# nyx-ai/droneRL

Hardware: AMD Instinct MI355X
Metric: env-steps/sec (obs/s) at num_envs=65536, 1/2/4/8 MI355X; %HBM roofline (higher is better)
Workload: dtype u8

## Files before the change

dronerl_amd/csrc/dronerl_internal.h:

```cpp
#pragma once
#include <hip/hip_runtime.h>
#include <stdint.h>

#include "../../include/dronerl.h"

namespace drl {

constexpr int MT_N = 624;
constexpr int MT_M = 397;
constexpr int MT_WORDS = DRL_MT_WORDS;
constexpr int MT_ALT = DRL_MT_BLOCK1;
constexpr int MT_RING = DRL_MT_RING;
constexpr int CAND_Q = DRL_CAND_SLOTS;
constexpr int MT_RING_END = DRL_MT_RING_END;
static_assert((CAND_Q & (CAND_Q - 1)) == 0 && CAND_Q <= 512, "ring size");
static_assert(MT_RING_END < MT_WORDS && MT_RING + CAND_Q <= MT_RING_END && MT_WORDS % 16 == 0, "MT row layout");

__host__ __device__ constexpr int mi_idx(uint32_t w) { return (int)(w & 0x3ffu); }
__host__ __device__ constexpr int mi_par(uint32_t w) { return (int)((w >> 10) & 1u); }
__host__ __device__ constexpr int mi_head(uint32_t w) { return (int)((w >> 11) & (uint32_t)(CAND_Q - 1)); }
__host__ __device__ constexpr int mi_cnt(uint32_t w) {
    return (int)((w >> 20) & 0x3ffu) < CAND_Q ? (int)((w >> 20) & 0x3ffu) : CAND_Q;
}
__host__ __device__ constexpr uint32_t mi_pack(int idx, int par, int head, int cnt) {
    return (uint32_t)idx | ((uint32_t)par << 10) | ((uint32_t)head << 11) | ((uint32_t)cnt << 20);
}
__host__ __device__ constexpr int ce_cell(uint32_t e) { return (int)(e & 0x3fffu); }
__host__ __device__ constexpr int ce_idx(uint32_t e) { return (int)((e >> 16) & 0x3ffu); }
__host__ __device__ constexpr int ce_par(uint32_t e) { return (int)((e >> 26) & 1u); }
__host__ __device__ constexpr uint32_t ce_pack(int cell, int idx, int par) {
    return (uint32_t)cell | ((uint32_t)idx << 16) | ((uint32_t)par << 26);
}
#ifndef DRL_CQ_NARROW
#define DRL_CQ_NARROW 2
#endif
constexpr int step_cq(int P) { return P <= 16 ? DRL_CQ_NARROW : 1; }
#ifndef DRL_DPP8
#define DRL_DPP8 1
#endif
#ifndef DRL_DRAWS_P8
#define DRL_DRAWS_P8 2
#endif
#ifndef DRL_DRAWS_P16
#define DRL_DRAWS_P16 2
#endif
#ifndef DRL_DRAWS_P32
#define DRL_DRAWS_P32 1
#endif
constexpr int step_draws(int P) {
    return P == 8 ? DRL_DRAWS_P8 : P == 16 ? DRL_DRAWS_P16 : P == 32 ? DRL_DRAWS_P32 : 1;
}
constexpr int kRolloutMinLanes = 16;
constexpr int kRolloutNoObsMinLanes = 8;
#ifndef DRL_ROLL_RING
#define DRL_ROLL_RING 1
#endif
#ifndef DRL_ROLL_RING_MAXP
#define DRL_ROLL_RING_MAXP 16
#endif
constexpr int OBS_U = 1;

namespace lay {
constexpr int r16(int v) { return (v + 15) / 16 * 16; }
constexpr int np(int n_drones) { return (n_drones + 7) / 8 * 8; }
constexpr int pstride(int side) { return r16((side * side + 1) / 2); }
constexpr int gstride(int side) { return 2 * pstride(side); }
#ifndef DRL_GL_NIB_MIN_SIDE
#define DRL_GL_NIB_MIN_SIDE 32
#endif
constexpr bool gl_nib(int side) { return side >= DRL_GL_NIB_MIN_SIDE; }
constexpr int glstride(int side) { return gl_nib(side) ? pstride(side) : gstride(side); }
constexpr int bm_bytes(int cells) { return r16((cells + 31) / 32 * 4); }
constexpr int paint_bytes(int k, int w) { return k > 0 ? r16(k * w * w) : 0; }
constexpr int nchg(int n_drones) { return 6 * n_drones + 2; }
constexpr int chg_bytes(int n_drones) { return r16(2 * nchg(n_drones)); }
constexpr int bit_length(int v) { return v ? 1 + bit_length(v >> 1) : 0; }
#ifndef DRL_QN_RING
#define DRL_QN_RING 2
#endif
#ifndef DRL_QN_WAVES
#define DRL_QN_WAVES 8
#endif
constexpr int code_cpg(int W) { return (W * W + 3) / 4; }
constexpr int code_cpg8(int W) { return (code_cpg(W) + 7) / 8 * 8; }
constexpr int code_bytes(int W) { return 4 * code_cpg8(W) * 2; }
constexpr int code_slot_cell(int cpg, int sl) { return sl < 6 * (cpg & ~1) ? 2 * (sl / 12) + (sl & 1) : cpg - 1; }
constexpr int code_slot_ch(int cpg, int sl) { return sl < 6 * (cpg & ~1) ? (sl % 12) / 2 : sl - 6 * (cpg - 1); }
constexpr int code_kt(int W) { return ((6 * code_cpg(W) + 7) / 8 + DRL_QN_RING - 1) / DRL_QN_RING * DRL_QN_RING; }
constexpr int qn_ring = DRL_QN_RING;
constexpr int qn_waves = DRL_QN_WAVES;
#ifndef DRL_QN_TILES
#define DRL_QN_TILES 2
#endif
constexpr int qn_tiles = DRL_QN_TILES;
constexpr int fy_bitmap_words(int cells) {
    int w = 64;
    while (w * 32 < cells) w *= 2;
    return w;
}
}

enum : int { OBJ_EMPTY = 0, OBJ_SKYSCRAPER = 2, OBJ_STATION = 3, OBJ_DROPZONE = 4, OBJ_PACKET = 5 };

struct FastDiv {
    uint32_t m;
    int one;
};

inline FastDiv make_fastdiv(uint32_t d) {
    FastDiv f;
    f.one = (d == 1);
    f.m = f.one ? 0u : (uint32_t)((((uint64_t)1 << 32) + d - 1) / d);
    return f;
}

struct ObsGeom {
    int side, radius;
    uint32_t W, per, env_floats, gstride;
    FastDiv div_env, div_per, div_6, div_w, div_side;
};

struct StepArgs {
    int side, n_drones, gstride, kbits;
    int pstride, gl_nib;
    int charge, discharge;
    float r_pickup, r_delivery, r_crash, r_charge;
    int64_t E;
    uint8_t* ground;
    uint32_t* drones;
    uint32_t* mt;
    uint32_t* mt_index;
    const int32_t* actions;
    float* rewards;
    uint8_t* dones;
    float* obs;
    int32_t* err;
    int wave_lds;
    int np;
    int lds_bm;
    int lds_paint;
    int lds_chg;
    int nchg;
    int obs_k;
    int obs_wide;
    int obs_nt;
    int specialize;
    int dones_packed;
    uint4* code;
    int code_lds;
    uint4* ring_obs;
    uint4* ring_next;
    int32_t* ring_act;
    float* ring_rew;
    uint8_t* ring_done;
    const uint4* code_prev;
    int64_t ring_first, ring_base, ring_cap;
    int synth;
    int64_t env_offset;
    uint64_t synth_seed, synth_step;
    uint32_t max_rounds;
    FastDiv div_side;
    ObsGeom og;
    int steps;
    int64_t act_tstride, out_tstride, obs_tstride;
};

struct RefillArgs {
    int side, kbits;
    int list;
    int64_t E;
    uint32_t* mt;
    uint32_t* mt_index;
};

struct ResetArgs {
    int side, n_drones, cells, gstride;
    int n_sky, n_pack, n_drop, n_stat;
    int64_t E;
    uint8_t* ground;
    uint32_t* drones;
    uint32_t* mt;
    uint32_t* mt_index;
    int reseed;
    uint64_t seed_base;
    const uint8_t* mask;
    int lanes, lane_lds, list_cap, block_lds, pool_branch;
    int wave_per_env, wave_lds;
    int wpb;
    int fy_batch_min;
    int fy_serial;
    int fy_bwords;
    FastDiv div_side;
};

constexpr int QN_MAX_LAYERS = 4;
struct QnetLayout {
    int n_layers;
    int nt[QN_MAX_LAYERS];
    int kt[QN_MAX_LAYERS];
    int in[QN_MAX_LAYERS], out[QN_MAX_LAYERS];
    int frag_off[QN_MAX_LAYERS];
    int bias_off[QN_MAX_LAYERS];
    int frag_total;
    int n_bias;
    int lds_vec;
    int precision;
    int frag_lo_off[QN_MAX_LAYERS];
    int total_vec;
    int frag_src[QN_MAX_LAYERS];
    int bias_vec;
    int lo0_lds;
    int code_w;
    int status_vec;
};

struct QnetPack {
    int n_layers;
    int frag_off[QN_MAX_LAYERS], kt[QN_MAX_LAYERS], in[QN_MAX_LAYERS], out[QN_MAX_LAYERS];
    int bias_off[QN_MAX_LAYERS];
    const float* w[QN_MAX_LAYERS];
    const float* b[QN_MAX_LAYERS];
    int64_t n_wfrag_elems, n_bias;
    uint16_t* packed_w;
    float* packed_b;
    int precision;
    int frag_lo_off[QN_MAX_LAYERS];
    int frag_src[QN_MAX_LAYERS];
    int code_w;
    int32_t* status;
};

struct QnetArgs {
    int in_features, kt0, n_hidden, n_actions, precision;
    const float* eps_ptr;
    int nt[QN_MAX_LAYERS];
    int frag_off[QN_MAX_LAYERS], bias_off[QN_MAX_LAYERS];
    int frag_total, lds_vec, n_bias;
    int frag_lo_off[QN_MAX_LAYERS];
    int bias_vec, lo0_lds;
    const uint4* packed;
    const float* obs;
    int64_t obs_stride, E;
    float epsilon;
    uint64_t seed, step;
    int64_t env_offset;
    int32_t* actions;
    int64_t action_stride;
    float* q;
    int synth_n;
    uint64_t synth_seed, synth_step;
    int32_t* err;
    int total_bytes;
    int status_vec;
};

struct ReplayArgs {
    int64_t first, n, cursor, capacity;
    int64_t base;
    int obs_floats;
    const float* obs;
    int64_t obs_stride;
    const float* next_obs;
    int64_t next_obs_stride;
    const int32_t* actions;
    int64_t action_stride;
    const float* rewards;
    int64_t reward_stride;
    const uint8_t* dones;
    int64_t done_stride;
    float* buf_obs;
    float* buf_next_obs;
    int32_t* buf_actions;
    float* buf_rewards;
    uint8_t* buf_dones;
};

__host__ __device__ constexpr int qn_frag_k(int g, int j) { return j < 4 ? 4 * g + j : 16 + 4 * g + (j - 4); }

struct PackSlot {
    int row, k;
};
__host__ __device__ inline PackSlot qnet_pack_slot(int l, int64_t e, int kt, int code_w, int in) {
    const int j = (int)(e & 7), lane = (int)((e >> 3) & 63);
    const int64_t frag = e >> 9;
    const int m = (int)(frag / kt), t = (int)(frag % kt);
    const int c = lane & 15, g = lane >> 4;
    PackSlot s{16 * m + c, 32 * t + qn_frag_k(g, j)};
    if (l == 0 && code_w > 0) {
        const int cpg = lay::code_cpg(code_w), cells = code_w * code_w, sl = 8 * t + j;
        const int lc = lay::code_slot_cell(cpg, sl), ch = lay::code_slot_ch(cpg, sl);
        const bool ok = sl < 6 * cpg && lc < cpg && g * cpg + lc < cells;
        s.k = ok ? (g * cpg + lc) * 6 + ch : in;
        if (g == 0 && sl == 6 * cpg) s.k = -1;
    }
    return s;
}

__host__ __device__ inline int64_t qnet_pack_elem(int l, int row, int k, int kt, int code_w) {
    int t, j, g;
    if (l == 0 && code_w > 0) {
        const int cpg = lay::code_cpg(code_w);
        int sl;
        if (k < 0) {
            g = 0;
            sl = 6 * cpg;
        } else {
            const int cell = k / 6, ch = k - 6 * cell;
            g = (cell >= cpg) + (cell >= 2 * cpg) + (cell >= 3 * cpg);
            const int lc = cell - g * cpg;
            sl = lc < (cpg & ~1) ? 12 * (lc / 2) + 2 * ch + (lc & 1) : 6 * (cpg - 1) + ch;
        }
        t = sl / 8;
        j = sl % 8;
    } else {
        t = k / 32;
        const int kk = k % 32;
        g = kk < 16 ? kk / 4 : (kk - 16) / 4;
        j = kk < 16 ? kk % 4 : 4 + (kk - 16) % 4;
    }
    const int m = row / 16, c = row % 16;
    return (((int64_t)m * kt + t) * 64 + (g * 16 + c)) * 8 + j;
}

__device__ __forceinline__ void qnet_pack_store(const QnetPack& p, int l, int64_t e, float w) {
    if (p.precision == DRL_QNET_F32) {
        if (!(__builtin_fabsf(w) < 65504.0f)) atomicOr(p.status, DRL_ERR_QNET_RANGE);
        const _Float16 hi = (_Float16)w;
        reinterpret_cast<_Float16*>(p.packed_w)[(int64_t)p.frag_off[l] * 8 + e] = hi;
        reinterpret_cast<_Float16*>(p.packed_w)[(int64_t)p.frag_lo_off[l] * 8 + e] = (_Float16)((w - (float)hi) * 2048.0f);
    } else {
        reinterpret_cast<__bf16*>(p.packed_w)[(int64_t)p.frag_off[l] * 8 + e] = (__bf16)w;
    }
}
__device__ __forceinline__ void qnet_pack_write(const QnetPack& p, int l, int64_t e, int k, float w) {
    if (l == 0 && p.code_w > 0 && k >= 0 && k < p.in[l] && k % 6 == 4) w /= 100.0f;
    qnet_pack_store(p, l, e, w);
}
__device__ __forceinline__ void qnet_pack_write_idx(const QnetPack& p, int l, uint32_t pe, float w) {
    if (pe >> 31) w /= 100.0f;
// ... 122 lines not shown
```

dronerl_amd/csrc/dronerl_kernels.hip:

```cpp
#include <hip/hip_runtime.h>
#include <stdint.h>

#include "dronerl_internal.h"
#include "dronerl_act_common.h"

namespace drl {

#ifdef DRL_STAMPS
__device__ unsigned long long* g_stamps;
#define DRL_STAMP(i)                                                                     \
    do {                                                                                 \
        __builtin_amdgcn_sched_barrier(0);                                               \
        unsigned long long t_;                                                           \
        asm volatile("s_memtime %0\n\ts_waitcnt lgkmcnt(0)" : "=s"(t_)::"memory");        \
        const int64_t sw_ = (int64_t)blockIdx.x * (blockDim.x >> 6) + (threadIdx.x >> 6); \
        if ((threadIdx.x & 63) == 0 && g_stamps) g_stamps[sw_ * 16 + (i)] = t_;          \
        if ((threadIdx.x & 63) == 0 && g_stamps && ((i) == 0 || (i) == 6))               \
            g_stamps[sw_ * 16 + 8 + (i) / 6] = __builtin_amdgcn_s_memrealtime();         \
        __builtin_amdgcn_sched_barrier(0);                                               \
    } while (0)
#define DRL_SUBT(v)                                                                  \
    do {                                                                             \
        __builtin_amdgcn_sched_barrier(0);                                           \
        asm volatile("s_memtime %0\n\ts_waitcnt lgkmcnt(0)" : "=s"(v)::"memory");   \
// ... 287 lines not shown
__device__ __forceinline__ uint32_t nib_get(const uint8_t* row, int cell) {
    return (row[cell >> 1] >> ((cell & 1) * 4)) & 15u;
}
__device__ __forceinline__ void nib_or(uint8_t* row, int cell, uint32_t code) {
    atomicOr(reinterpret_cast<uint32_t*>(row) + (cell >> 3), code << ((cell & 7) * 4));
}
__device__ __forceinline__ uint32_t nib_get_l2(uint8_t* row, int cell) {
    const uint32_t w = __hip_atomic_load(reinterpret_cast<uint32_t*>(row) + (cell >> 3), __ATOMIC_RELAXED,
                                         __HIP_MEMORY_SCOPE_AGENT);
    return (w >> ((cell & 7) * 4)) & 15u;
}
__device__ __forceinline__ void nib_clear(uint8_t* row, int cell) {
    atomicAnd(reinterpret_cast<uint32_t*>(row) + (cell >> 3), ~(15u << ((cell & 7) * 4)));
}

template <class GEO>
__device__ __forceinline__ int gl_get(const GEO& g, const l_u8* gl, int cell) {
    if (g.nib()) return (gl[cell >> 1] >> ((cell & 1) << 2)) & 15;
    return gl[cell];
}
template <class GEO>
__device__ __forceinline__ void gl_clear(const GEO& g, l_u8* gl, int cell) {
    if (g.nib()) __atomic_fetch_and(reinterpret_cast<l_u32*>(gl) + (cell >> 3), ~(15u << ((cell & 7) << 2)),
                                    __ATOMIC_RELAXED);
    else gl[cell] = OBJ_EMPTY;
}
template <class GEO>
__device__ __forceinline__ void gl_put(const GEO& g, l_u8* gl, int cell, int obj) {
    if (g.nib()) __atomic_fetch_or(reinterpret_cast<l_u32*>(gl) + (cell >> 3), (uint32_t)obj << ((cell & 7) << 2),
                                   __ATOMIC_RELAXED);
    else gl[cell] = (uint8_t)obj;
}

template <bool NT>
__device__ __forceinline__ void store_obs16(uint4* p, u32x4 v) {
    if constexpr (NT) {
        __builtin_nontemporal_store(v, reinterpret_cast<u32x4*>(p));
    } else {
        *reinterpret_cast<u32x4*>(p) = v;
    }
}

template <class T>
__device__ __forceinline__ void lds_zero(T* p, int nbytes, int lane) {
    l_u4* q = reinterpret_cast<l_u4*>(p);
    for (int v = lane; v < nbytes / 16; v += 64) q[v] = (u32x4){0u, 0u, 0u, 0u};
}

template <bool NT = false, bool CODE = false, bool F32 = true, class GEO>
__device__ __forceinline__ void write_obs_wave(float* __restrict__ base, int nenv_w, const GEO& g, const WaveLds& w,
                                               bool obs_wide, int lane, uint16_t* __restrict__ code = nullptr,
                                               l_u16* cst = nullptr) {
    static_assert(CODE || F32, "nothing to write");
    const uint32_t W = g.W();
    const uint32_t win = W * W;
    const uint32_t env_cells = g.env_cells();
    const uint32_t ncell = (uint32_t)nenv_w * env_cells;
    const int G = g.side(), R = g.radius();
    const uint32_t gstride = (uint32_t)g.gstride(), np = (uint32_t)g.np(), lpaint = (uint32_t)g.lds_paint();
    const bool wide = obs_wide && ((uintptr_t)base & 15u) == 0;
    const int cpg = lay::code_cpg((int)W), cpg8 = lay::code_cpg8((int)W);
    if constexpr (CODE) {
        lds_zero(cst, nenv_w * 8 * cpg8, lane);
        wave_sync();
    }
    for (uint32_t q0 = 0; q0 < ncell; q0 += 64 * OBS_U) {
        uint32_t e[OBS_U], rem[OBS_U], wy[OBS_U], wx[OBS_U], pos[OBS_U];
#pragma unroll
        for (int u = 0; u < OBS_U; ++u) {
            const uint32_t q = min(q0 + (uint32_t)(lane + 64 * u), ncell - 1u);
            e[u] = g.div_env(q);
            rem[u] = q - e[u] * env_cells;
            const uint32_t k = g.div_win(rem[u]);
            const uint32_t c = rem[u] - k * win;
            wy[u] = g.div_w(c);
            wx[u] = c - wy[u] * W;
            pos[u] = w.posidx[e[u] * np + k];
        }
        float2 v[OBS_U][3];
#pragma unroll
        for (int u = 0; u < OBS_U; ++u) {
            const uint32_t py = g.div_side(pos[u]);
            const uint32_t px = pos[u] - py * (uint32_t)G;
            const int y = (int)(py + wy[u]) - R;
            const int x = (int)(px + wx[u]) - R;
            const bool in = (unsigned)y < (unsigned)G && (unsigned)x < (unsigned)G;
            const uint32_t o = (uint32_t)gl_get(g, w.gl + e[u] * gstride, in ? y * G + x : 0);
            const uint32_t obj = in ? o : (uint32_t)OBJ_SKYSCRAPER;
            const uint32_t air = w.paint[e[u] * lpaint + rem[u]];
            if constexpr (CODE) {
                if (rem[u] < win) {
                    const uint32_t cl = rem[u], grpc = cl / (uint32_t)cpg;
                    cst[e[u] * (uint32_t)(4 * cpg8) + grpc * (uint32_t)(cpg8 - cpg) + cl] = (uint16_t)(obj | (air << 3));
                }
            }
            if constexpr (!F32) continue;
            v[u][0].x = air ? 1.0f : 0.0f;
            v[u][0].y = (obj == OBJ_PACKET || (air & 0x80u)) ? 1.0f : 0.0f;
            v[u][1].x = obj == OBJ_DROPZONE ? 1.0f : 0.0f;
            v[u][1].y = obj == OBJ_STATION ? 1.0f : 0.0f;
            v[u][2].x = air ? div100((int)(air & 0x7fu) - 1) : 0.0f;
            v[u][2].y = obj == OBJ_SKYSCRAPER ? 1.0f : 0.0f;
        }
        if constexpr (!F32) continue;
        if (wide) {
            l_f2* st = reinterpret_cast<l_f2*>(w.stage);
#pragma unroll
            for (int u = 0; u < OBS_U; ++u) {
                const int slot = (u * 64 + lane) * 3;
                st[slot] = (f32x2){v[u][0].x, v[u][0].y};
                st[slot + 1] = (f32x2){v[u][1].x, v[u][1].y};
                st[slot + 2] = (f32x2){v[u][2].x, v[u][2].y};
            }
            wave_sync();
            const l_u4* sv = reinterpret_cast<const l_u4*>(w.stage);
            uint4* dst = reinterpret_cast<uint4*>(base + 6u * q0);
            if (q0 + 64u * OBS_U <= ncell) {
#pragma unroll
                for (int t = 0; t < 96 * OBS_U; t += 64)
                    if (96 * OBS_U - t >= 64 || lane < 96 * OBS_U - t) store_obs16<NT>(&dst[t + lane], sv[t + lane]);
            } else {
                const uint32_t nbytes = (ncell - q0) * 24u;
                for (uint32_t t = lane; t * 16u < nbytes; t += 64) {
                    if (t * 16u + 16u <= nbytes) {
                        store_obs16<NT>(&dst[t], sv[t]);
                    } else {
                        reinterpret_cast<u32x2*>(dst + t)[0] = reinterpret_cast<const l_u2*>(sv + t)[0];
                    }
                }
            }
            wave_sync();
        } else {
#pragma unroll
            for (int u = 0; u < OBS_U; ++u) {
                const uint32_t q = q0 + (uint32_t)(lane + 64 * u);
                if (q < ncell) {
                    float2* o = reinterpret_cast<float2*>(base + 6u * q);
                    o[0] = v[u][0];
                    o[1] = v[u][1];
                    o[2] = v[u][2];
                }
            }
        }
    }
    if constexpr (CODE) {
        wave_sync();
        const l_u4* cv = reinterpret_cast<const l_u4*>(cst);
        uint4* dst = reinterpret_cast<uint4*>(code);
        for (int v = lane; v < nenv_w * cpg8 / 2; v += 64) {
            const u32x4 x = cv[v];
            dst[v] = make_uint4(x[0], x[1], x[2], x[3]);
        }
    }
}

template <class GEO>
__device__ __forceinline__ uint16_t* code_row(const StepArgs& a, int64_t wenv0, const GEO& g) {
    return reinterpret_cast<uint16_t*>(a.code) + wenv0 * (int64_t)(4 * lay::code_cpg8((int)g.W()));
}

template <class A>
__device__ __forceinline__ int64_t step_ring_slot(const A& a, int64_t e) {
    const int64_t s = a.ring_base + (e - a.ring_first);
    return s >= a.ring_cap ? s - a.ring_cap : s;
}

template <class A>
__device__ __forceinline__ bool ring_vec(const A& a, int64_t wenv0, uint32_t v, uint32_t VR, int64_t* e,
                                         uint32_t* col) {
    const uint32_t el = v / VR;
    *col = v - el * VR;
    *e = wenv0 + el;
    return *e >= a.ring_first;
}

template <int RQ, class A>
__device__ __forceinline__ void step_ring_prefetch(const A& a, int64_t wenv0, int nenv_w, int lane, uint32_t VR,
                                                   u32x4 (&pre)[RQ]) {
    const uint32_t nv = (uint32_t)nenv_w * VR;
#pragma unroll
    for (int q = 0; q < RQ; ++q) {
        const uint32_t v = (uint32_t)(lane + 64 * q);
        int64_t e;
        uint32_t col;
        if (v < nv && ring_vec(a, wenv0, v, VR, &e, &col))
            pre[q] = reinterpret_cast<const u32x4*>(a.code_prev)[e * VR + col];
    }
}

template <int RQ, class A>
__device__ __forceinline__ void step_ring_sink(const A& a, int64_t wenv0, int nenv_w, const l_u16* cst,
                                               int lane, uint32_t VR, const u32x4 (&pre)[RQ]) {
    const l_u4* cv = reinterpret_cast<const l_u4*>(cst);
    const uint32_t nv = (uint32_t)nenv_w * VR;
#pragma unroll
    for (int q = 0; q < RQ; ++q) {
        const uint32_t v = (uint32_t)(lane + 64 * q);
        int64_t e;
        uint32_t col;
        if (v < nv && ring_vec(a, wenv0, v, VR, &e, &col)) {
            const int64_t slot = step_ring_slot(a, e);
            const u32x4 next = cv[v];
            __builtin_nontemporal_store(next, reinterpret_cast<u32x4*>(a.ring_next) + slot * VR + col);
            __builtin_nontemporal_store(pre[q], reinterpret_cast<u32x4*>(a.ring_obs) + slot * VR + col);
        }
    }
    for (uint32_t v = (uint32_t)(lane + 64 * RQ); v < nv; v += 64) {
        int64_t e;
        uint32_t col;
        if (!ring_vec(a, wenv0, v, VR, &e, &col)) continue;
        const int64_t slot = step_ring_slot(a, e);
        const u32x4 prev = reinterpret_cast<const u32x4*>(a.code_prev)[e * VR + col];
        const u32x4 next = cv[v];
        __builtin_nontemporal_store(next, reinterpret_cast<u32x4*>(a.ring_next) + slot * VR + col);
        __builtin_nontemporal_store(prev, reinterpret_cast<u32x4*>(a.ring_obs) + slot * VR + col);
    }
}

template <class GEO>
__device__ __forceinline__ void paint_windows(l_u8* paint, const l_u16* posidx, int y, int x, uint8_t airbyte,
                                              const GEO& g) {
    const int W = (int)g.W(), K = g.K(), R = g.radius();
    for (int k = 0; k < K; ++k) {
        const uint32_t pk = posidx[k];
        const int pky = (int)g.div_side(pk);
        const int pkx = (int)pk - pky * g.side();
        const int dy = y - pky + R, dx = x - pkx + R;
        if ((unsigned)dy < (unsigned)W && (unsigned)dx < (unsigned)W) paint[k * W * W + dy * W + dx] = airbyte;
    }
}

__device__ __forceinline__ void chg_push(const WaveLds& w, int grp, int nchg_cap, int cell) {
    const uint32_t q = __atomic_fetch_add(&w.cnt[grp * 4], 1u, __ATOMIC_RELAXED);
    if (q < (uint32_t)nchg_cap) w.chg[grp * nchg_cap + q] = (uint16_t)cell;
}

__device__ __forceinline__ bool bm_test(const l_u32* bm, int cell) { return (bm[cell >> 5] >> (cell & 31)) & 1u; }
__device__ __forceinline__ void bm_set(l_u32* bm, int cell) { __atomic_fetch_or(&bm[cell >> 5], 1u << (cell & 31), __ATOMIC_RELAXED); }

template <int P> struct GMaskT { using type = uint32_t; };
template <> struct GMaskT<64> { using type = uint64_t; };

template <int P>
__device__ __forceinline__ typename GMaskT<P>::type gballot(bool pred, int gshift) {
    using M = typename GMaskT<P>::type;
    const uint64_t b = __ballot(pred);
    if constexpr (P == 64) return b;
    else return (M)(b >> gshift) & (M)((1ull << P) - 1ull);
}
__device__ __forceinline__ int popc(uint32_t m) { return __popc(m); }
__device__ __forceinline__ int popc(uint64_t m) { return __popcll(m); }
__device__ __forceinline__ int lobit(uint32_t m) { return __ffs(m) - 1; }
__device__ __forceinline__ int lobit(uint64_t m) { return __ffsll((unsigned long long)m) - 1; }
__device__ __forceinline__ int hibit(uint32_t m) { return 31 - __clz(m); }
__device__ __forceinline__ int hibit(uint64_t m) { return 63 - __clzll((long long)m); }

template <int P>
__device__ __forceinline__ int gshfl(int v, int src, int lane) {
#ifdef DRL_HIP_SHFL
    return __shfl(v, src, P);
#else
    return __builtin_amdgcn_ds_bpermute(((lane & ~(P - 1)) + (src & (P - 1))) << 2, v);
#endif
}

template <int P>
__device__ __forceinline__ int gbase(int lane) {
    int b = (lane & ~(P - 1)) << 2;
    asm volatile("" : "+v"(b));
    return b;
}
template <int P>
__device__ __forceinline__ int gshfl_at(int v, int base, int src) {
    return __builtin_amdgcn_ds_bpermute(base + ((src & (P - 1)) << 2), v);
}

template <int K>
__device__ __forceinline__ int xor_lane8(int v) {
    if constexpr (K == 1) return __builtin_amdgcn_update_dpp(0, v, 0xB1, 0xf, 0xf, false);
    else if constexpr (K == 2) return __builtin_amdgcn_update_dpp(0, v, 0x4E, 0xf, 0xf, false);
    else if constexpr (K == 3) return __builtin_amdgcn_update_dpp(0, v, 0x1B, 0xf, 0xf, false);
    else if constexpr (K == 7) return __builtin_amdgcn_update_dpp(0, v, 0x141, 0xf, 0xf, false);
    else return __builtin_amdgcn_update_dpp(0, xor_lane8<K ^ 7>(v), 0x141, 0xf, 0xf, false);
}
template <int K>
__device__ __forceinline__ int xor_lane16(int v) {
    if constexpr (K < 8) return xor_lane8<K>(v);
    else return __builtin_amdgcn_update_dpp(0, xor_lane8<K ^ 15>(v), 0x140, 0xf, 0xf, false);
}
template <int P, int K = 1, class F>
__device__ __forceinline__ void for_other_lanes(int v, F&& f) {
    if constexpr (K < P) {
        f(P == 8 ? xor_lane8<K>(v) : xor_lane16<K>(v), K);
        for_other_lanes<P, K + 1>(v, f);
    }
}

template <int P, class GEO, bool ROLL, bool NT, bool CODE = false, bool RING = false>
__device__ __forceinline__ void step_batch(const StepArgs& a, int64_t wenv0) {
    using GMask = typename GMaskT<P>::type;
    constexpr int GPW = 64 / P;
    static_assert(!ROLL || P >= kRolloutNoObsMinLanes, "narrow groups roll out as drl_step launches");
    constexpr int D = step_draws(P);
    constexpr int QL = step_cq(P);
    using CM = typename GMaskT<(P * D <= 32 ? 32 : 64)>::type;
#ifndef DRL_SHFL_BATCH
#define DRL_SHFL_BATCH 16
#endif
    constexpr int CH = P < DRL_SHFL_BATCH ? P : DRL_SHFL_BATCH;
    extern __shared__ __attribute__((aligned(16))) unsigned char smem_all[];
    unsigned char* const smem = smem_all + (size_t)__builtin_amdgcn_readfirstlane(threadIdx.x >> 6) *
                                               (size_t)((a.wave_lds + 15) & ~15);
    const GEO g{a};
    const int lane0 = threadIdx.x & 63;
    const int grp0 = lane0 / P;
    const int j0 = lane0 % P;
    const int nenv_w = (int)min((int64_t)GPW, a.E - wenv0);
    if (nenv_w <= 0) return;
    const bool env_ok0 = grp0 < nenv_w;
    const int G = g.side(), N = g.n(), gstride = g.gstride(), nchg = g.nchg();
    const WaveLds W = carve((l_u8*)smem, GPW, P, g);
    uint32_t* const drones_w = a.drones + wenv0 * N;
    uint32_t* const mt_w = a.mt + wenv0 * MT_WORDS;
    const int pstride = g.pstride();
    uint8_t* const ground_w = a.ground + wenv0 * pstride;
    const uint32_t rl0 = (uint32_t)(grp0 * N);

    DRL_STAMP(0);
    uint32_t mi[GPW];
#pragma unroll
    for (int e = 0; e < GPW; ++e) mi[e] = a.mt_index[wenv0 + min(e, nenv_w - 1)];
    lds_zero(W.bm, GPW * g.lds_bm(), lane0);
    if (GEO::kObs && (a.obs || CODE)) lds_zero(W.paint, GPW * g.lds_paint(), lane0);
    if (lane0 < GPW) W.cnt[lane0 * 4] = 0u;
    wave_sync();
    const bool active0 = env_ok0 && j0 < N;
    const uint32_t li0 = min(rl0 + (uint32_t)j0, (uint32_t)(nenv_w * N - 1));
    const uint32_t rec_ld = drones_w[li0];
#ifdef DRL_DIAG_ACT_U8
    const int act_ld = reinterpret_cast<const uint8_t*>(a.actions)[wenv0 * N + li0] % 5;
#else
    const int act_ld = a.actions[(RING && a.synth) ? (wenv0 + min(grp0, nenv_w - 1)) * (int64_t)N
                                                   : wenv0 * N + li0];
#endif
    [[maybe_unused]] NibStage<(GEO::kPstride > 0 ? GPW * GEO::kPstride / 16 : 1), (GEO::kGstride == GEO::kPstride)> nib;
    if constexpr (GEO::kPstride > 0) nib.load(ground_w, nenv_w * pstride, lane0);
    else stage_ground_nib(ground_w, nenv_w * pstride, W.gl, lane0, g.nib());
    __builtin_amdgcn_sched_barrier(0);
    [[maybe_unused]] int syn_act = 0;
    if constexpr (RING) {
        if (a.synth) syn_act = synth_action(a.synth_seed, a.synth_step, (uint64_t)(a.env_offset + wenv0 + grp0),
                                            (uint64_t)j0);
    }
    uint32_t mword = mi[0];
#pragma unroll
    for (int e = 1; e < GPW; ++e) mword = (grp0 >= e) ? mi[e] : mword;
    uint32_t rec = active0 ? rec_ld : 0u;
    int my_action = active0 ? act_ld : 4;
    if constexpr (RING) {
        if (a.synth && j0 != 0 && active0) my_action = syn_act;
    }
    if (!env_ok0) mword = (uint32_t)MT_N;
    int midx = 0;
    l_u32* const stash = W.stash;
    constexpr bool kRing = !ROLL || (DRL_ROLL_RING && P >= kRolloutMinLanes && P <= DRL_ROLL_RING_MAXP);
    uint32_t cq[QL];
    auto ring_issue = [&](const uint32_t mw) __attribute__((always_inline)) {
        const uint32_t rbase = (uint32_t)(env_ok0 ? grp0 : 0) * MT_WORDS + MT_RING;
        const int qh = mi_head(mw);
#pragma unroll
#ifdef DRL_DIAG_RING_FIXED
        for (int r = 0; r < QL; ++r) cq[r] = mt_w[MT_RING + ((j0 + P * r) & (CAND_Q - 1))];
#else
        for (int r = 0; r < QL; ++r) cq[r] = mt_w[rbase + ((qh + j0 + P * r) & (CAND_Q - 1))];
#endif
    };
    int act_next = 4;
    const int T = ROLL ? a.steps : 1;
    for (int t = 0; t < T; ++t) {
    const int lane = lane0, grp = lane / P, j = lane % P;
    const bool env_ok = grp < nenv_w;
    const bool active = env_ok && j < N;
    const uint32_t rl = (uint32_t)(grp * N);
    const uint32_t li = min(rl + (uint32_t)j, (uint32_t)(nenv_w * N - 1));
    l_u8* gl = W.gl + grp * gstride;
    l_u32* bm = W.bm + grp * (g.lds_bm() / 4);
    l_u16* posidx = W.posidx + grp * g.np();
    const uint32_t* mrow = mt_w + (uint32_t)(env_ok ? grp : 0) * MT_WORDS;
    if constexpr (ROLL) {
        if (t > 0) {
            rec = active ? stash[lane] : 0u;
            my_action = active ? act_next : 4;
            wave_sync();
            lds_zero(W.bm, GPW * g.lds_bm(), lane);
            if (GEO::kObs && a.obs) lds_zero(W.paint, GPW * g.lds_paint(), lane);
            wave_sync();
        }
        if (t + 1 < T) act_next = a.actions[(t + 1) * a.act_tstride + wenv0 * N + li];
    }

#ifdef DRL_NIB_EARLY
    if constexpr (GEO::kGstride > 0 && !ROLL) {
        if (g.nib()) nib.store(W.gl, lane0, true);
    }
#endif
    DRL_STAMP(1);
    const int y = rec & 255u, x = (rec >> 8) & 255u;
    const int idx = ((int)(rec >> 25) < N) ? (int)(rec >> 25) : j;
    int c = (rec >> 16) & 255u;
    int carry = (rec >> 24) & 1u;
    int act;
    act = gshfl<P>(my_action, idx, lane);
    __builtin_amdgcn_sched_barrier(0);
    if constexpr (kRing) ring_issue(mword);
    [[maybe_unused]] uint32_t pfq[ROLL ? D : 1];
    [[maybe_unused]] bool pf_live = false;
    if constexpr (ROLL) {
        pf_live = (!kRing || mi_cnt(mword) == 0) && mi_idx(mword) + D * P <= MT_N;
        const uint32_t* src = mt_w + (uint32_t)(env_ok ? grp : 0) * MT_WORDS + (uint32_t)mi_par(mword) * MT_ALT;
#pragma unroll
        for (int q = 0; q < D; ++q) pfq[q] = load_l2(src + min(mi_idx(mword) + q * P + j, MT_N - 1));
    }
    __builtin_amdgcn_sched_barrier(0);
    if (active) {
        if (act < 0) act += 5;
        if ((unsigned)act > 4u) {
            if (a.err) atomicOr(a.err, DRL_ERR_BAD_ACTION);
            act = 4;
        }
    }
    const int ty = y + (act == 1) - (act == 3);
    const int tx = x + (act == 2) - (act == 0);
    const bool inb = active && ty >= 0 && ty < G && tx >= 0 && tx < G;
    const int tcell = inb ? ty * G + tx : -1 - j;

    bool earlier = false;
    int later_min = P;
    if constexpr ((P == 8 || P == 16) && DRL_DPP8) {
        for_other_lanes<P>(tcell, [&](int o, int k) {
            const int s = j ^ k;
            const bool same = o == tcell;
            earlier |= same && s < j;
            later_min = (same && s > j && s < later_min) ? s : later_min;
        });
    } else {
    const int gb = gbase<P>(lane);
#pragma unroll
    for (int s0 = 0; s0 < P; s0 += CH) {
        int ts[CH];
#pragma unroll
        for (int t = 0; t < CH; ++t) ts[t] = gshfl_at<P>(tcell, gb, s0 + t);
#pragma unroll
        for (int t = 0; t < CH; ++t) {
            const int s = s0 + t;
            const bool same = ts[t] == tcell;
            earlier |= same && s < j;
            later_min = (same && s > j && s < later_min) ? s : later_min;
        }
    }
    }
    const bool claimer = inb && !earlier;
    const bool crashA = active && !claimer;
    if constexpr (GEO::kGstride > 0) {
#ifdef DRL_NIB_EARLY
        if (t == 0 && (ROLL || !g.nib())) nib.store(W.gl, lane0, g.nib());
#else
        if (t == 0) nib.store(W.gl, lane0, g.nib());
#endif
    }
    wave_sync();

    DRL_STAMP(2);
    float reward = 0.0f;
    bool dead = false, deliver = false;
    if (claimer) {
        const int obj = gl_get(g, gl, tcell);
        if (obj == OBJ_STATION) {
            c = min(100, c + a.charge);
            reward = a.r_charge;
        } else {
            c -= a.discharge;
            dead = c <= 0;
        }
        if (obj == OBJ_PACKET && !carry) {
            reward = a.r_pickup;
            carry = 1;
            gl_clear(g, gl, tcell);
            if constexpr (!ROLL) chg_push(W, grp, nchg, tcell);
        } else if (obj == OBJ_DROPZONE && carry) {
            reward = a.r_delivery;
            carry = 0;
            gl_clear(g, gl, tcell);
            deliver = true;
            if constexpr (!ROLL) chg_push(W, grp, nchg, tcell);
        }
        if (obj == OBJ_SKYSCRAPER) dead = true;
    }

    const bool collided = claimer && later_min < P;
    const bool crashB = claimer && (collided || dead);
    const bool survivor = claimer && !crashB;
    const bool crashed = crashA || crashB;
    const int gshift = grp * P;
    const uint64_t gm = (P == 64) ? ~0ull : (((1ull << (P & 63)) - 1ull) << gshift);
    const uint64_t lower = (1ull << lane) - 1ull;
    const uint64_t bS = __ballot(survivor) & gm;
    const uint64_t bA = __ballot(crashA) & gm;
    const uint64_t bB = __ballot(crashB) & gm;
    const int nS = __popcll(bS), nA = __popcll(bA), nR = nA + __popcll(bB);
    int rankB = 0;
    if (__ballot(crashB)) {
        const int bkey = crashB ? (collided ? later_min : P + j) : 4 * P;
        if constexpr ((P == 8 || P == 16) && DRL_DPP8) {
            for_other_lanes<P>(bkey, [&](int o, int) { rankB += o < bkey; });
        } else {
        const int gb = gbase<P>(lane);
#pragma unroll
        for (int s0 = 0; s0 < P; s0 += CH) {
            int ks[CH];
#pragma unroll
            for (int t = 0; t < CH; ++t) ks[t] = gshfl_at<P>(bkey, gb, s0 + t);
#pragma unroll
            for (int t = 0; t < CH; ++t) rankB += (ks[t] < bkey);
        }
        }
    }
    const int newslot = survivor ? __popcll(bS & lower)
                                 : (crashA ? nS + __popcll(bA & lower) : (crashB ? nS + nA + rankB : j));
    const int n_deliver = __popcll(__ballot(deliver) & gm);
    const int n_pack = n_deliver + __popcll(__ballot(crashed && carry) & gm);
    const int total = nR + n_pack + n_deliver;
    if (crashed) {
        c = 100;
        carry = 0;
        reward = a.r_crash;
    }
    int pos = survivor ? tcell : -1;
    if (survivor) bm_set(bm, tcell);
    wave_sync();

    DRL_STAMP(3);
#ifdef DRL_DIAG_NO_RESPAWN
    int w = total, have_y = 0, yv = 0;
#else
    int w = 0, have_y = 0, yv = 0;
#endif
    const int shift = 32 - g.kbits();
    const int my_item = crashed ? newslot - nS : -1;
    {
        const int qcnt = (kRing && env_ok) ? mi_cnt(mword) : 0;
        const int GGc = G * G;
        int start = 0;
        uint32_t ent_last = 0;
        auto batch = [&](const uint32_t cqr, const int r) __attribute__((always_inline)) {
            const int cell = ce_cell(cqr);
            const bool valid = env_ok && P * r + j < qcnt && cell < GGc;
            const int ccell = valid ? cell : 0;
            const int tg = valid ? cell : -1 - j;
            int prev = -1;
            if constexpr ((P == 8 || P == 16) && DRL_DPP8) {
                for_other_lanes<P>(tg, [&](int o, int k) {
                    const int s2 = j ^ k;
                    prev = (o == tg && s2 < j && s2 > prev) ? s2 : prev;
                });
            } else {
                const int gb = gbase<P>(lane);
#pragma unroll
                for (int s0 = 0; s0 < P; s0 += CH) {
                    int ts[CH];
#pragma unroll
                    for (int t2 = 0; t2 < CH; ++t2) ts[t2] = gshfl_at<P>(tg, gb, s0 + t2);
#pragma unroll
                    for (int t2 = 0; t2 < CH; ++t2) prev = (ts[t2] == tg && s0 + t2 < j) ? s0 + t2 : prev;
                }
            }
            const int gobj = gl_get(g, gl, ccell);
            const bool occ = bm_test(bm, ccell);
            const int bend = min(P * (r + 1), qcnt);
#pragma unroll
            for (int cs = 0; cs < 3; ++cs) {
                const bool act = env_ok && w < total && start < bend;
                if (!__ballot(act)) break;
                const bool isd = w < nR;
                const int cls_end = isd ? nR : (w < nR + n_pack ? nR + n_pack : total);
                const int need = cls_end - w;
                const int gnow = cs == 0 ? gobj : gl_get(g, gl, ccell);
                const bool fresh = valid && P * r + j >= start && (prev < 0 || P * r + prev < start);
                const bool ok = act && fresh && (isd ? (!occ && gnow != OBJ_SKYSCRAPER) : gnow == OBJ_EMPTY);
                const GMask M = gballot<P>(ok, gshift);
                const int k = min(popc(M), need);
                const int rank = popc(M & ((GMask(1) << j) - GMask(1)));
                const bool chosen = ok && rank < k;
                const GMask C = gballot<P>(chosen, gshift);
                if (chosen) {
                    if (isd) {
                        posidx[w + rank] = (uint16_t)cell;
                        bm_set(bm, cell);
                    } else {
                        gl_put(g, gl, cell, (w + rank < nR + n_pack) ? OBJ_PACKET : OBJ_DROPZONE);
                        if constexpr (!ROLL) chg_push(W, grp, nchg, cell);
                    }
                }
                const bool done = k == need;
                const uint32_t el = (uint32_t)gshfl<P>((int)cqr, done ? hibit(C) : bend - 1 - P * r, lane);
                if (act) {
                    start = done ? P * r + hibit(C) + 1 : bend;
                    ent_last = el;
                    w += k;
                }
                wave_sync();
            }
        };
        if constexpr (kRing) {
#pragma unroll
            for (int r = 0; r < QL; ++r) {
                if (!__ballot(env_ok && w < total && start < qcnt)) break;
                batch(cq[r], r);
            }
            for (int r = QL; r < CAND_Q / P; ++r) {
                if (!__ballot(env_ok && w < total && start < qcnt)) break;
                const uint32_t* ring = mt_w + (uint32_t)(env_ok ? grp : 0) * MT_WORDS + MT_RING;
                batch(ring[(mi_head(mword) + j + P * r) & (CAND_Q - 1)], r);
            }
        }
        if (crashed && my_item < w) pos = posidx[my_item];
        const bool dry = env_ok && w < total;
        const int ncons = start;
        const uint32_t ent = ent_last;
        midx = min(ncons > 0 ? ce_idx(ent) : mi_idx(mword), MT_N);
        const int mpar = ncons > 0 ? ce_par(ent) : mi_par(mword);
        const uint32_t nword = mi_pack(midx, mpar, (mi_head(mword) + ncons) & (CAND_Q - 1), qcnt - ncons);
        if constexpr (ROLL) {
            if (!dry) mword = nword;
        } else if (env_ok && j == 0 && !dry) {
            W.cnt[grp * 4 + 1] = nword;
        }
        mrow += (uint32_t)mpar * MT_ALT;
        wave_sync();
    }
    uint32_t rounds = 0;
    [[maybe_unused]] uint32_t rounds_w = 0;
    [[maybe_unused]] unsigned long long sub_t0 = 0, sub_t1 = 0, sub_t2 = 0, sub_t3 = 0, sub_acc[4] = {0, 0, 0, 0};
    for (;;) {
        const bool work = env_ok && w < total;
        if (!__ballot(work)) break;
        ++rounds_w;
        DRL_SUBT(sub_t0);
        uint64_t need = __ballot(work && j == 0 && midx >= MT_N);
        while (need) {
            const int tl = __ffsll((unsigned long long)need) - 1;
            need &= need - 1ull;
#ifndef DRL_DIAG_NO_TWIST
            {
                const uint64_t pr = (uint64_t)(uintptr_t)mrow;
                const uint64_t lo = (uint32_t)__builtin_amdgcn_readlane((int)(uint32_t)pr, tl);
                const uint64_t hi = (uint32_t)__builtin_amdgcn_readlane((int)(uint32_t)(pr >> 32), tl);
                twist_wave(reinterpret_cast<uint32_t*>((hi << 32) | lo), lane);
            }
#endif
            if (grp == tl / P) midx = 0;
        }
        DRL_SUBT(sub_t1);
        const int avail = MT_N - midx;
        int rq[D], ccq[D];
        bool candq[D], accq[D];
        GMask mq[D];
        CM accall = 0;
#pragma unroll
        for (int q = 0; q < D; ++q) {
            const int d = q * P + j;
            const bool valid = work && d < avail;
            uint32_t word = 0u;
            if constexpr (ROLL) word = pfq[q];
            if (__ballot(valid && !pf_live)) word = (valid && !pf_live) ? load_l2(mrow + midx + d) : word;
            rq[q] = valid ? (int)(temper(word) >> shift) : G;
            accq[q] = rq[q] < G;
            mq[q] = gballot<P>(accq[q], gshift);
            accall |= CM(mq[q]) << (q * P);
        }
        auto r_at = [&](int b) {
            int v = gshfl<P>(rq[0], b % P, lane);
#pragma unroll
            for (int q = 1; q < D; ++q) {
                const int vq = gshfl<P>(rq[q], b % P, lane);
                v = (b / P == q) ? vq : v;
            }
            return v;
        };
        GMask okd = 0, okg = 0;
        CM okdc = 0, okgc = 0;
#pragma unroll
        for (int q = 0; q < D; ++q) {
            const CM prevm = accall & ((CM(1) << (q * P + j)) - CM(1));
            const int apos = have_y + popc(prevm);
            const int pl = prevm ? hibit(prevm) : 0;
            const int rp = r_at(pl);
            const int ycand = prevm ? rp : yv;
            candq[q] = accq[q] && (apos & 1);
            ccq[q] = candq[q] ? ycand * G + rq[q] : 0;
            const int gobj = gl_get(g, gl, ccq[q]);
            const bool occ = bm_test(bm, ccq[q]);
            okd = gballot<P>(candq[q] && !occ && gobj != OBJ_SKYSCRAPER, gshift);
            okg = gballot<P>(candq[q] && gobj == OBJ_EMPTY, gshift);
            okdc |= CM(okd) << (q * P);
            okgc |= CM(okg) << (q * P);
        }
        DRL_SUBT(sub_t2);
        int last = -1;
        bool more = work;
#ifdef DRL_DIAG_NO_PLACE
        if (more) {
            const CM m0 = (w < nR ? okdc : okgc);
            last = m0 ? lobit(m0) : D * P - 1;
            pos = (my_item >= 0 && m0) ? ccq[0] : pos;
            w = m0 ? total : w;
            more = false;
        }
#endif
        while (__ballot(more)) {
            if (more) {
                const bool isd = w < nR;
                const CM after = (last < 0) ? ~CM(0) : ~((CM(2) << last) - CM(1));
                const CM m = (isd ? okdc : okgc) & after;
                if (!m) {
                    more = false;
                } else {
                    const int b = lobit(m);
                    int cell = gshfl<P>(ccq[0], b % P, lane);
#pragma unroll
                    for (int q = 1; q < D; ++q) {
                        const int cq = gshfl<P>(ccq[q], b % P, lane);
                        cell = (b / P == q) ? cq : cell;
                    }
                    CM same = 0;
#pragma unroll
                    for (int q = 0; q < D; ++q) same |= CM(gballot<P>(candq[q] && ccq[q] == cell, gshift)) << (q * P);
                    if (isd) {
                        pos = (my_item == w) ? cell : pos;
                        if (j == 0) bm_set(bm, cell);
                        okdc &= ~same;
                    } else {
                        if (j == 0) {
                            gl_put(g, gl, cell, (w < nR + n_pack) ? OBJ_PACKET : OBJ_DROPZONE);
                            if constexpr (!ROLL) chg_push(W, grp, nchg, cell);
                        }
                        okgc &= ~same;
                    }
                    last = b;
                    ++w;
                    more = w < total;
                }
            }
        }
        DRL_SUBT(sub_t3);
        if constexpr (ROLL) pf_live = false;
        if (work) {
            if (w >= total) {
                midx += last + 1;
                have_y = 0;
            } else {
                const int cnt = have_y + popc(accall);
                const int yl = r_at(accall ? hibit(accall) : 0);
                if (accall && (cnt & 1)) yv = yl;
                have_y = cnt & 1;
                midx += min(D * P, avail);
            }
            if (++rounds > a.max_rounds) {
                if (j == 0 && a.err) atomicOr(a.err, DRL_ERR_NO_FREE_CELL);
                w = total;
                if (crashed && pos < 0) pos = 0;
            }
        }
        wave_sync();
#ifdef DRL_STAMPS
        {
            unsigned long long t4;
            DRL_SUBT(t4);
            sub_acc[3] += t4 - sub_t3;
        }
        sub_acc[0] += sub_t1 - sub_t0;
        sub_acc[1] += sub_t2 - sub_t1;
        sub_acc[2] += sub_t3 - sub_t2;
#endif
    }
#ifdef DRL_STAMPS
    if (lane == 0)
        for (int k = 0; k < 4; ++k)
            if (g_stamps) g_stamps[((int64_t)blockIdx.x * (blockDim.x >> 6) + (threadIdx.x >> 6)) * 16 + 10 + k] = sub_acc[k];
#endif

    DRL_STAMP(4);
#ifdef DRL_STAMPS
    if (lane == 0 && g_stamps) g_stamps[((int64_t)blockIdx.x * (blockDim.x >> 6) + (threadIdx.x >> 6)) * 16 + 7] = __builtin_amdgcn_readfirstlane(rounds_w);
#endif
    if (active && pos < 0) pos = 0;
    if (active && !carry && gl_get(g, gl, pos) == OBJ_PACKET) {
        carry = 1;
        gl_clear(g, gl, pos);
        if constexpr (!ROLL) chg_push(W, grp, nchg, pos);
    }

    const uint32_t py = g.div_side((uint32_t)(pos > 0 ? pos : 0));
    const uint32_t px = (uint32_t)(pos > 0 ? pos : 0) - py * (uint32_t)G;
    const uint32_t rec_out = pack_drone((int)py, (int)px, c, carry, idx);
    const bool dpack = a.dones_packed;
    l_u8* const dn = reinterpret_cast<l_u8*>(bm);
    if (active) {
        if constexpr (!ROLL) drones_w[rl + newslot] = rec_out;
        a.rewards[t * a.out_tstride + wenv0 * N + (rl + idx)] = reward;
        if constexpr (RING) {
            const StepArgs& ka = *(const StepArgs*)__builtin_amdgcn_kernarg_segment_ptr();
            const int64_t e = wenv0 + grp;
            if (idx == 0 && e >= ka.ring_first) {
                const int64_t slot = step_ring_slot(ka, e);
                ka.ring_act[slot] = ka.actions[e * N];
                ka.ring_rew[slot] = reward;
                ka.ring_done[slot] = crashed ? 1 : 0;
            }
        }
#ifndef DRL_DIAG_NO_SMALL_WB
        if (dpack) dn[idx] = crashed ? 1 : 0;
        else a.dones[t * a.out_tstride + wenv0 * N + (rl + idx)] = crashed ? 1 : 0;
#endif
        posidx[idx] = (uint16_t)pos;
    }
    if constexpr (ROLL) {
        if (rounds > 0) mword = mi_pack(midx, mrow != mt_w + (uint32_t)(env_ok ? grp : 0) * MT_WORDS ? 1 : 0, 0, 0);
    } else if (env_ok && j == 0) {
#ifdef DRL_DIAG_NO_SMALL_WB
        if (a.E < 0)
#endif
        a.mt_index[wenv0 + grp] = rounds > 0 ? mi_pack(midx, mrow != mt_w + (uint32_t)grp * MT_WORDS ? 1 : 0, 0, 0)
                                             : W.cnt[grp * 4 + 1];
    }
    wave_sync();
    if (dpack && env_ok && j < (N >> 2))
        reinterpret_cast<uint32_t*>(a.dones + t * a.out_tstride + wenv0 * N + rl)[j] =
            reinterpret_cast<const l_u32*>(dn)[j];
    if (!ROLL && env_ok) {
        const uint32_t nc = W.cnt[grp * 4];
        const l_u16* ch = W.chg + grp * nchg;
        uint8_t* gdst = ground_w + (uint32_t)(grp * pstride);
#ifndef DRL_DIAG_NO_GROUND_WB
#pragma clang loop unroll(disable) vectorize(disable)
        for (uint32_t q = j; q < min(nc, (uint32_t)nchg); q += P) {
            const uint32_t e = ch[q] & ~1u;
            gdst[e >> 1] = g.nib() ? gl[e >> 1] : (uint8_t)(gl[e] | (gl[e + 1] << 4));
        }
#endif
    }
    DRL_STAMP(5);
    if (GEO::kObs && (a.obs || (CODE && !ROLL))) {
        const StepArgs& ka = *(const StepArgs*)__builtin_amdgcn_kernarg_segment_ptr();
        constexpr int RQ = RING ? (GPW * (GEO::kW > 1 ? lay::code_cpg8((int)GEO::kW) / 2 : 12) + 63) / 64 : 1;
        const uint32_t VR = (uint32_t)lay::code_cpg8((int)g.W()) / 2u;
        [[maybe_unused]] u32x4 rpre[RQ];
        if constexpr (RING) step_ring_prefetch<RQ>(ka, wenv0, nenv_w, lane, VR, rpre);
        if (active) paint_windows(W.paint + grp * g.lds_paint(), posidx, (int)py, (int)px,
                                  (uint8_t)((c + 1) | (carry << 7)), g);
        wave_sync();
        float* obase = a.obs + t * a.obs_tstride + wenv0 * (int64_t)(6u * g.env_cells());
        if constexpr (CODE && !ROLL) {
            uint16_t* crow = code_row(a, wenv0, g);
            l_u16* cst = reinterpret_cast<l_u16*>((l_u8*)smem + a.code_lds);
            if (a.obs) write_obs_wave<NT, true, true>(obase, nenv_w, g, W, a.obs_wide, lane, crow, cst);
            else write_obs_wave<NT, true, false>(obase, nenv_w, g, W, a.obs_wide, lane, crow, cst);
            if constexpr (RING) step_ring_sink<RQ>(ka, wenv0, nenv_w, cst, lane, VR, rpre);
        } else {
            write_obs_wave<NT>(obase, nenv_w, g, W, a.obs_wide, lane);
        }
    }
    DRL_STAMP(6);
    if constexpr (ROLL) {
        wave_sync();
        if (active) stash[grp * P + newslot] = rec_out;
    }
    }
    if constexpr (ROLL) {
        wave_sync();
        if (active0) drones_w[rl0 + j0] = stash[lane0];
        if (env_ok0 && j0 == 0) a.mt_index[wenv0 + grp0] = mword;
        uint4* dst = reinterpret_cast<uint4*>(ground_w);
        for (int v = lane0; v < nenv_w * pstride / 16; v += 64) {
            if (g.nib()) {
                const u32x4 x = reinterpret_cast<const l_u4*>(W.gl)[v];
                dst[v] = make_uint4(x[0], x[1], x[2], x[3]);
            } else {
                dst[v] = nib_pack_load(W.gl + v * 32);
            }
        }
    }
}

#ifndef DRL_XCD_REMAP
#define DRL_XCD_REMAP 0
#endif
__device__ __forceinline__ uint32_t xcd_block(uint32_t orig, uint32_t n) {
    if (!DRL_XCD_REMAP) return orig;
    const uint32_t q = n / 8, r = n % 8, x = orig % 8;
    return (x < r ? x * (q + 1) : r * (q + 1) + (x - r) * q) + orig / 8;
}

#ifndef DRL_STEP_WAVES_P16
#define DRL_STEP_WAVES_P16 6
#endif
#ifndef DRL_STEP_WAVES_P32
#define DRL_STEP_WAVES_P32 1
#endif
#ifndef DRL_STEP_WPB_P16
#define DRL_STEP_WPB_P16 1
#endif
#ifndef DRL_STEP_WPB_P32
#define DRL_STEP_WPB_P32 1
#endif
constexpr int step_wpb(int P) { return P == 32 ? DRL_STEP_WPB_P32 : P == 16 ? DRL_STEP_WPB_P16 : 1; }
template <int P, class GEO, bool NT, bool CODE = false, bool RING = false>
__global__ void __launch_bounds__(64 * step_wpb(P))
__attribute__((amdgpu_waves_per_eu(P <= 8 ? 8 : (P == 32 ? DRL_STEP_WAVES_P32 : P == 16 ? DRL_STEP_WAVES_P16 : 1), 8)))
drl_step_kernel(StepArgs a) {
    constexpr int WPB = step_wpb(P);
    const int64_t batch = WPB == 1 ? (int64_t)xcd_block(blockIdx.x, gridDim.x)
                                   : (int64_t)blockIdx.x * WPB + __builtin_amdgcn_readfirstlane(threadIdx.x >> 6);
    step_batch<P, GEO, false, NT, CODE, RING>(a, batch * (64 / P));
}

// ... 1050 lines not shown
```

Before: 3.261 billion.

## Issue candidate ring prefetch early and size first ring window per group width

Adds a configurable first ring window (WIN) per group width and generalizes the batch lambda to take a base offset and length. For non-rollout steps with pstride geometries it hoists the candidate-ring loads before the step loop, behind a scheduling barrier, so their latency overlaps earlier work. It also clamps ring load offsets to the valid candidate count, avoiding reads past the live queue. This can change register pressure and adds partial-window batches, for example P=16 now prefetches only one batch instead of two.

Result: no change. 3.278 billion, median of 6 (+0.5%).

```diff
diff --git a/dronerl_amd/csrc/dronerl_internal.h b/dronerl_amd/csrc/dronerl_internal.h
--- a/dronerl_amd/csrc/dronerl_internal.h
+++ b/dronerl_amd/csrc/dronerl_internal.h
@@ -35,6 +35,18 @@
 #define DRL_CQ_NARROW 2
 #endif
 constexpr int step_cq(int P) { return P <= 16 ? DRL_CQ_NARROW : 1; }
+#ifndef DRL_RING_WIN_P8
+#define DRL_RING_WIN_P8 (8 * step_cq(8))
+#endif
+#ifndef DRL_RING_WIN_P16
+#define DRL_RING_WIN_P16 16
+#endif
+#ifndef DRL_RING_WIN_P32
+#define DRL_RING_WIN_P32 (32 * step_cq(32))
+#endif
+constexpr int step_win(int P) {
+    return P == 8 ? DRL_RING_WIN_P8 : P == 16 ? DRL_RING_WIN_P16 : P == 32 ? DRL_RING_WIN_P32 : P * step_cq(P);
+}
 #ifndef DRL_DPP8
 #define DRL_DPP8 1
 #endif
diff --git a/dronerl_amd/csrc/dronerl_kernels.hip b/dronerl_amd/csrc/dronerl_kernels.hip
--- a/dronerl_amd/csrc/dronerl_kernels.hip
+++ b/dronerl_amd/csrc/dronerl_kernels.hip
@@ -613,7 +613,9 @@
     constexpr int GPW = 64 / P;
     static_assert(!ROLL || P >= kRolloutNoObsMinLanes, "narrow groups roll out as drl_step launches");
     constexpr int D = step_draws(P);
-    constexpr int QL = step_cq(P);
+    constexpr int WIN = ROLL ? P * step_cq(P) : step_win(P);
+    static_assert(WIN >= 1 && WIN <= P * step_cq(P), "the first ring window lies within the lanes' batches");
+    constexpr int QL = (WIN + P - 1) / P;
     using CM = typename GMaskT<(P * D <= 32 ? 32 : 64)>::type;
 #ifndef DRL_SHFL_BATCH
 #define DRL_SHFL_BATCH 16
@@ -679,13 +681,22 @@
     auto ring_issue = [&](const uint32_t mw) __attribute__((always_inline)) {
         const uint32_t rbase = (uint32_t)(env_ok0 ? grp0 : 0) * MT_WORDS + MT_RING;
         const int qh = mi_head(mw);
-#pragma unroll
+        [[maybe_unused]] const int qlast = min(WIN, max(mi_cnt(mw), 1)) - 1;
+#pragma unroll
+        for (int r = 0; r < QL; ++r) {
+            const int off = ROLL ? j0 + P * r : min(j0 + P * r, qlast);
 #ifdef DRL_DIAG_RING_FIXED
-        for (int r = 0; r < QL; ++r) cq[r] = mt_w[MT_RING + ((j0 + P * r) & (CAND_Q - 1))];
+            cq[r] = mt_w[MT_RING + (min(j0 + P * r, WIN - 1) & (CAND_Q - 1))];
 #else
-        for (int r = 0; r < QL; ++r) cq[r] = mt_w[rbase + ((qh + j0 + P * r) & (CAND_Q - 1))];
-#endif
+            cq[r] = mt_w[rbase + ((qh + off) & (CAND_Q - 1))];
+#endif
+        }
     };
+    constexpr bool kRingEarly = kRing && !ROLL && GEO::kPstride > 0;
+    if constexpr (kRingEarly) {
+        ring_issue(mword);
+        __builtin_amdgcn_sched_barrier(0);
+    }
     int act_next = 4;
     const int T = ROLL ? a.steps : 1;
     for (int t = 0; t < T; ++t) {
@@ -723,7 +734,7 @@
     int act;
     act = gshfl<P>(my_action, idx, lane);
     __builtin_amdgcn_sched_barrier(0);
-    if constexpr (kRing) ring_issue(mword);
+    if constexpr (kRing && !kRingEarly) ring_issue(mword);
     [[maybe_unused]] uint32_t pfq[ROLL ? D : 1];
     [[maybe_unused]] bool pf_live = false;
     if constexpr (ROLL) {
@@ -863,9 +874,9 @@
         const int GGc = G * G;
         int start = 0;
         uint32_t ent_last = 0;
-        auto batch = [&](const uint32_t cqr, const int r) __attribute__((always_inline)) {
+        auto batch = [&](const uint32_t cqr, const int base, const int len) __attribute__((always_inline)) {
             const int cell = ce_cell(cqr);
-            const bool valid = env_ok && P * r + j < qcnt && cell < GGc;
+            const bool valid = env_ok && j < len && base + j < qcnt && cell < GGc;
             const int ccell = valid ? cell : 0;
             const int tg = valid ? cell : -1 - j;
             int prev = -1;
@@ -887,7 +898,7 @@
             }
             const int gobj = gl_get(g, gl, ccell);
             const bool occ = bm_test(bm, ccell);
-            const int bend = min(P * (r + 1), qcnt);
+            const int bend = min(base + len, qcnt);
 #pragma unroll
             for (int cs = 0; cs < 3; ++cs) {
                 const bool act = env_ok && w < total && start < bend;
@@ -896,7 +907,7 @@
                 const int cls_end = isd ? nR : (w < nR + n_pack ? nR + n_pack : total);
                 const int need = cls_end - w;
                 const int gnow = cs == 0 ? gobj : gl_get(g, gl, ccell);
-                const bool fresh = valid && P * r + j >= start && (prev < 0 || P * r + prev < start);
+                const bool fresh = valid && base + j >= start && (prev < 0 || base + prev < start);
                 const bool ok = act && fresh && (isd ? (!occ && gnow != OBJ_SKYSCRAPER) : gnow == OBJ_EMPTY);
                 const GMask M = gballot<P>(ok, gshift);
                 const int k = min(popc(M), need);
@@ -913,9 +924,9 @@
                     }
                 }
                 const bool done = k == need;
-                const uint32_t el = (uint32_t)gshfl<P>((int)cqr, done ? hibit(C) : bend - 1 - P * r, lane);
+                const uint32_t el = (uint32_t)gshfl<P>((int)cqr, done ? hibit(C) : bend - 1 - base, lane);
                 if (act) {
-                    start = done ? P * r + hibit(C) + 1 : bend;
+                    start = done ? base + hibit(C) + 1 : bend;
                     ent_last = el;
                     w += k;
                 }
@@ -926,12 +937,13 @@
 #pragma unroll
             for (int r = 0; r < QL; ++r) {
                 if (!__ballot(env_ok && w < total && start < qcnt)) break;
-                batch(cq[r], r);
-            }
-            for (int r = QL; r < CAND_Q / P; ++r) {
+                batch(cq[r], P * r, P * (r + 1) <= WIN ? P : WIN - P * r);
+            }
+            for (int base = WIN; base < CAND_Q; base += P) {
                 if (!__ballot(env_ok && w < total && start < qcnt)) break;
                 const uint32_t* ring = mt_w + (uint32_t)(env_ok ? grp : 0) * MT_WORDS + MT_RING;
-                batch(ring[(mi_head(mword) + j + P * r) & (CAND_Q - 1)], r);
+                const int off = ROLL ? base + j : min(base + j, max(qcnt, 1) - 1);
+                batch(ring[(mi_head(mword) + off) & (CAND_Q - 1)], base, P);
             }
         }
         if (crashed && my_item < w) pos = posidx[my_item];
```
